# mitenjain/nanopore

Hardware: AMD Instinct MI355X
Metric: DP cells/sec (banded pair-HMM realign: forward + backward + posterior per cell) (higher is better)
Workload: dtype f32

## Files before the change

### nanopore_amd/csrc/npr_api.cpp

```cpp
#include "npr_api_internal.h"

namespace npr_impl {
DeviceArena g_arena[kMaxDevices];
}

extern "C" {

int32_t npr_abi_version(void) { return NPR_ABI_VERSION; }

const char *npr_strerror(int32_t code) {
    switch (code) {
        case NPR_OK: return "ok";
        case NPR_ERR_INVALID: return "invalid argument or guide alignment not global";
        case NPR_ERR_ZERO_PROB: return "total probability is zero inside the band";
        case NPR_ERR_CAPACITY: return "output capacity exceeded";
        case NPR_ERR_MODEL: return "unsupported or malformed HMM";
        case NPR_ERR_NO_DEVICE: return "no usable gfx950 device (there is no CPU fallback)";
        case NPR_ERR_HIP: return "HIP runtime error";
        case NPR_ERR_BAND_TOO_WIDE: return "band wider than the kernels support";
        case NPR_ERR_NOMEM: return "out of memory";
        case NPR_ERR_STATE: return "call sequence violated";
        default: return "unknown error";
    }
}
// ... 34 lines not shown
    }
    npr_ctx *ctx = new (std::nothrow) npr_ctx;
    if (!ctx) return NPR_ERR_NOMEM;
    ctx->device = device_id;
    ctx->arena = &g_arena[device_id];
    {
        std::lock_guard<std::mutex> lock(ctx->arena->mu);
        ++ctx->arena->users;
    }
    ctx->cu_count = prop.multiProcessorCount;
    ctx->total_mem = prop.totalGlobalMem;
    ctx->host_threads = usable_cpus();
    int prio_lo = 0, prio_hi = 0;
    (void)hipDeviceGetStreamPriorityRange(&prio_lo, &prio_hi);
    for (int i = 0; i < npr_ctx::kSideStreams; ++i)
        if ((e = hipStreamCreateWithPriority(&ctx->side[i], hipStreamNonBlocking, prio_hi)) != hipSuccess ||
            (e = hipEventCreateWithFlags(&ctx->side_done[i], hipEventDisableTiming)) != hipSuccess) {
            say("npr_create: side stream allocation", e);
            npr_destroy(ctx);
            return NPR_ERR_HIP;
        }
    if ((e = hipStreamCreateWithFlags(&ctx->stream, hipStreamNonBlocking)) != hipSuccess ||
        (e = hipEventCreate(&ctx->ev0)) != hipSuccess || (e = hipEventCreate(&ctx->ev1)) != hipSuccess ||
        (e = hipMalloc(reinterpret_cast<void **>(&ctx->d_models), sizeof(DevModel) * NPR_MAX_MODELS)) != hipSuccess) {
        say("npr_create: stream/event/model allocation", e);
        npr_destroy(ctx);
        return NPR_ERR_HIP;
    }
    const int32_t rc = npr_set_hmm(ctx, 0, nullptr, nullptr);
    if (rc != NPR_OK) {
        if (err && errlen) std::snprintf(err, errlen, "npr_create: %s", ctx->last_error.c_str());
        npr_destroy(ctx);
        return rc;
    }
    *out = ctx;
    return NPR_OK;
}

void npr_destroy(npr_ctx *ctx) {
    if (!ctx) return;
    (void)hipSetDevice(ctx->device);
    ctx->cache_flush();
    if (ctx->d_models) (void)hipFree(ctx->d_models);
    if (ctx->arena) {
        std::lock_guard<std::mutex> lock(ctx->arena->mu);
        if (--ctx->arena->users == 0) {
            if (ctx->arena->F) (void)hipFree(ctx->arena->F - DeviceArena::kPad);
            ctx->arena->F = nullptr, ctx->arena->cells = 0, ++ctx->arena->epoch;
        }
    }
    if (ctx->arena_Fx) (void)hipFree(reinterpret_cast<char *>(ctx->arena_Fx) - npr_ctx::kArenaPad);
    if (ctx->pin_pairs) (void)hipHostFree(ctx->pin_pairs);
    if (ctx->pin_stage) (void)hipHostFree(ctx->pin_stage);
    delete ctx->mea;
    for (hipEvent_t ev : ctx->ops_events) (void)hipEventDestroy(ev);
    if (ctx->ev0) (void)hipEventDestroy(ctx->ev0);
    if (ctx->ev1) (void)hipEventDestroy(ctx->ev1);
    if (ctx->stream) (void)hipStreamDestroy(ctx->stream);
    for (int i = 0; i < npr_ctx::kSideStreams; ++i) {
        if (ctx->side[i]) (void)hipStreamDestroy(ctx->side[i]);
        if (ctx->side_done[i]) (void)hipEventDestroy(ctx->side_done[i]);
    }
    delete ctx;
}

const char *npr_last_error(npr_ctx *ctx) { return ctx ? ctx->last_error.c_str() : ""; }

}
namespace npr_impl {
int32_t release_scratch(npr_ctx *ctx, bool caches_only) {
    HIP_TRY(ctx, hipSetDevice(ctx->device));
    HIP_TRY(ctx, hipStreamSynchronize(ctx->stream));
    ctx->cache_flush();
    if (caches_only) return NPR_OK;
    if (ctx->arena) {
        std::lock_guard<std::mutex> lock(ctx->arena->mu);
        if (ctx->arena->F) (void)hipFree(ctx->arena->F - DeviceArena::kPad);
        ctx->arena->F = nullptr, ctx->arena->cells = 0, ++ctx->arena->epoch;
    }
    if (ctx->arena_Fx) (void)hipFree(reinterpret_cast<char *>(ctx->arena_Fx) - npr_ctx::kArenaPad);
    ctx->arena_Fx = nullptr, ctx->arena_fx_cells = 0;
    delete ctx->mea;
    ctx->mea = nullptr;
    ctx->packed_pool.clear();
    return NPR_OK;
}
}
extern "C" {

int32_t npr_ctx_option(npr_ctx *ctx, int32_t option, int64_t value) {
    if (!ctx) return NPR_ERR_INVALID;
    switch (option) {
        case NPR_OPT_OVERLAP: ctx->overlap = value == 2 ? 2 : (value != 0 ? 1 : 0); return NPR_OK;
        case NPR_OPT_RELEASE_SCRATCH: return release_scratch(ctx, value == 2);
        case 10: case 11: case 12: case 16: case 18: case 19: break;
        default:
            if (option > NPR_OPT_RELEASE_SCRATCH && option < NPR_OPT_COUNT) {
                ctx->opt[option] = value;
                return NPR_OK;
            }
    }
    return fail(ctx, NPR_ERR_INVALID, "npr_ctx_option: unknown option");
}

int32_t npr_set_hmm(npr_ctx *ctx, int32_t slot, const double *T25, const double *E80) {
    if (!ctx || slot < 0 || slot >= NPR_MAX_MODELS) return NPR_ERR_INVALID;
// ... 139 lines not shown
```

### nanopore_amd/csrc/npr_api_internal.h

```cpp
#pragma once
#include <hip/hip_runtime.h>

#include <algorithm>
#include <atomic>
#include <chrono>
#include <cmath>
#include <cstdio>
#include <cstdlib>
#include <cstring>
#include <exception>
#include <memory>
#include <mutex>
#include <new>
#include <numeric>
#include <string>
#include <thread>
#include <type_traits>
#include <vector>

#include "npr_device.h"
#include "npr_internal.h"
#include "npr_sched.h"
#include "npr_threads.h"

using namespace npr;

struct npr_plan {
    Plan plan;
};

namespace npr_impl {
struct MeaScratch;

struct DeviceArena {
    static constexpr size_t kPad = 1024;
    std::mutex mu;
    char *F = nullptr;
    std::atomic<size_t> cells{0};
    std::atomic<uint64_t> epoch{1};
    int users = 0;
};
constexpr int kMaxDevices = 64;
extern DeviceArena g_arena[kMaxDevices];
}
using namespace npr_impl;

struct npr_ctx {
    int device = -1;
    hipStream_t stream = nullptr;
    hipEvent_t ev0 = nullptr, ev1 = nullptr;
    static constexpr int kSideStreams = 6;
    hipStream_t side[kSideStreams] = {};
    hipEvent_t side_done[kSideStreams] = {};
    int cu_count = 0;
    size_t total_mem = 0;
    bool model_set[NPR_MAX_MODELS] = {};
    DevModel models[NPR_MAX_MODELS];
    DevModel *d_models = nullptr;
    std::string last_error;
    int host_threads = 1;
    DeviceArena *arena = nullptr;
    int overlap = 0;
    int64_t opt[NPR_OPT_COUNT] = {};
    static constexpr size_t kArenaPad = DeviceArena::kPad;
    float *arena_Fx = nullptr;
    size_t arena_fx_cells = 0;
    void *pin_pairs = nullptr;
    size_t pin_pairs_bytes = 0;
    std::vector<hipEvent_t> ops_events;
    struct HostWords {
        std::unique_ptr<uint32_t[]> p;
        int64_t cap = 0;
    };
    std::vector<HostWords> packed_pool;
    void *pin_stage = nullptr;
    size_t pin_stage_bytes = 0;
    MeaScratch *mea = nullptr;
    struct Cached {
        void *p;
        size_t bytes;
    };
    std::vector<Cached> cache;
    size_t cache_bytes = 0;
    void cache_flush() {
        for (const Cached &c : cache) (void)hipFree(c.p);
        cache.clear();
        cache_bytes = 0;
    }
};

namespace npr_impl {

inline int poison_byte() {
    const char *e = std::getenv("NPR_POISON");
    return e && e[0] ? static_cast<int>(std::strtol(e, nullptr, 0)) & 0xff : -1;
}
inline void poison(void *p, size_t bytes) {
    if (poison_byte() >= 0 && p && bytes) {
        (void)hipMemset(p, poison_byte(), bytes);
        (void)hipDeviceSynchronize();
    }
}

template <typename T>
struct DevBuf {
    T *p = nullptr;
    size_t count = 0, cap = 0;
    hipError_t alloc(size_t n) {
        release();
        count = n;
        if (n == 0) return hipSuccess;
        const hipError_t e = hipMalloc(reinterpret_cast<void **>(&p), n * sizeof(T));
        if (e == hipSuccess) poison(p, n * sizeof(T));
        return e;
    }
    void release() {
        if (p && !borrowed) {
            if (owner && owner->cache.size() < 160) {
                owner->cache.push_back(npr_ctx::Cached{p, held});
                owner->cache_bytes += held;
            } else {
                (void)hipFree(p);
            }
        }
        p = nullptr;
        count = 0, cap = 0, borrowed = false, owner = nullptr, held = 0;
    }
    bool borrowed = false;
    void borrow(T *ptr, size_t n) {
        release();
        p = ptr, count = n, borrowed = true;
    }
    size_t bytes() const { return count * sizeof(T); }
    npr_ctx *owner = nullptr;
    size_t held = 0;
    hipError_t alloc_from(npr_ctx *ctx, size_t n) {
        release();
        count = n;
        if (n == 0) return hipSuccess;
        const size_t need = n * sizeof(T);
        constexpr size_t kSmall = size_t(1) << 20, kPiece = size_t(256) << 10;
        int best = -1;
        for (size_t i = 0; i < ctx->cache.size(); ++i)
            if (ctx->cache[i].bytes >= need && (ctx->cache[i].bytes <= 2 * need || ctx->cache[i].bytes <= kSmall) &&
                (best < 0 || ctx->cache[i].bytes < ctx->cache[best].bytes))
                best = static_cast<int>(i);
        if (best >= 0) {
            p = static_cast<T *>(ctx->cache[best].p), held = ctx->cache[best].bytes, owner = ctx;
            ctx->cache_bytes -= held;
            ctx->cache.erase(ctx->cache.begin() + best);
            poison(p, held);
            return hipSuccess;
        }
        const size_t take = need < kSmall ? (need + kPiece - 1) / kPiece * kPiece : need + need / 8;
        hipError_t e = hipMalloc(reinterpret_cast<void **>(&p), take);
        if (e != hipSuccess && !ctx->cache.empty()) {
            (void)hipGetLastError();
            ctx->cache_flush();
            e = hipMalloc(reinterpret_cast<void **>(&p), take);
        }
        if (e == hipSuccess) held = take, owner = ctx, poison(p, take);
        return e;
    }
    hipError_t reserve(size_t n) {
        if (n <= cap && p) {
            count = n;
            return hipSuccess;
        }
        const hipError_t e = alloc(n + n / 4 + 1);
        cap = e == hipSuccess ? count : 0;
        count = e == hipSuccess ? n : 0;
        return e;
    }
    ~DevBuf() { release(); }
};

struct MeaScratch {
    DevBuf<int64_t> off, mass, od;
    DevBuf<int32_t> cnt, start, col, sorted, small, tmp, map, pieces;
    DevBuf<uint32_t> dense;
};

inline int32_t fail(npr_ctx *ctx, int32_t code, const char *what, hipError_t e = hipSuccess) {
    if (code == NPR_ERR_HIP && e == hipErrorOutOfMemory) code = NPR_ERR_NOMEM, (void)hipGetLastError();
    if (ctx) {
        ctx->last_error = what;
        if (e != hipSuccess) {
            ctx->last_error += ": ";
            ctx->last_error += hipGetErrorString(e);
        }
    }
    return code;
}

#define HIP_TRY(ctx, expr)                                                  \
    do {                                                                    \
        hipError_t _e = (expr);                                             \
        if (_e != hipSuccess) return fail((ctx), NPR_ERR_HIP, #expr, _e);   \
    } while (0)

struct StageTimer {
    bool on;
    std::chrono::steady_clock::time_point t0;
    const char *what;
    explicit StageTimer(const char *w) : on(std::getenv("NPR_TIMING") != nullptr), t0(std::chrono::steady_clock::now()), what(w) {}
    void lap(const char *label) {
        if (!on) return;
        const auto t1 = std::chrono::steady_clock::now();
        std::fprintf(stderr, "[npr timing] %s / %s: %.1f ms\n", what, label, std::chrono::duration<double, std::milli>(t1 - t0).count());
        t0 = t1;
    }
};

}
using namespace npr_impl;

struct npr_batch {
    npr_ctx *ctx = nullptr;
    npr_params params{};
    int64_t n_reads = 0;
    std::vector<int64_t> ref_len, read_len;
    std::vector<int64_t> gstart;
    std::vector<int32_t> ref_id;
    std::vector<int32_t> guide_ops;
    std::vector<int64_t> guide_off;
    std::vector<int32_t> read_status;
    std::vector<int32_t> read_first_task, read_ntasks;
    std::vector<Task> tasks;
    std::vector<int32_t> task_of;
    std::vector<int64_t> task_cells;
    std::vector<TaskOut> outs;
    std::vector<uint8_t> task_rerun;
// ... 167 lines not shown
```

### nanopore_amd/csrc/npr_device.h

```cpp
#pragma once
#include <cstdint>

#include "npr_internal.h"
#include "npr_band.h"

namespace npr {

struct Task {
    int64_t x_off;
    int64_t y_off;
    int64_t band_off;
    int64_t pair_off;
    int32_t lX, lY;
    int32_t D;
    int32_t pair_cap;
    int32_t flags;
    int32_t model;
    int32_t xs, ys;
    int32_t read;
    int32_t cells_pad;
    int64_t ctl_off;
    int64_t tile_off;
    int64_t rowmask_off;
};
// ... 56 lines not shown
    const int32_t *px;
    const int32_t *py;
    const float *pp;
    int32_t *cx;
    int32_t *cy;
    float *cp;
};

int launch_generic(const KernelArgs &a, int grid, int threads, size_t lds_bytes, bool dense, bool global_ring, void *stream);
int launch_em(const KernelArgs &a, int grid, size_t lds_bytes, bool global_ring, void *stream);
size_t em_extra_lds_bytes();
int launch_compact(const CompactArgs &a, void *stream);
int launch_stair(const KernelArgs &a, int R, int grid, void *stream);
int launch_wide(const KernelArgs &a, int R, int NW, int grid, void *stream);
int launch_em_stair(const KernelArgs &a, int R, int grid, void *stream);
size_t em_stair_lds_bytes();
struct MeaArgs {
    const Task *tasks;
    const TaskOut *outs;
    int32_t ntasks, n_reads;
    const int32_t *px, *py;
    const float *pp;
    const int64_t *rx_off;
    const int64_t *ry_off;
    const int64_t *rp_off;
    int32_t *cnt, *start, *colsum;
    int32_t *sx, *sy, *sq, *back;
    int32_t *kx, *ky, *kq, *kback;
    int4 *vrec;
    int32_t *kept;
    const int32_t *np, *poff, *pboff, *lane_read, *lane_piece;
    int32_t *pb, *pbest;
    int32_t n_pieces;
    int32_t *best_who;
    int32_t *read_flag;
    double gap_gamma, match_gamma;
    int32_t ring;
    const int32_t *order;
    const int32_t *read_first, *read_ntasks, *task_of;
    int32_t sort_lds_bytes;
    int32_t sort_threads;
    int32_t any_global_sort;
    const int64_t *cnt_off;
    int32_t ring_only;
    int32_t *ops_tmp;
    const int64_t *ot_off;
    int32_t *n_ops, *chain_len;
    int64_t *chain_mass;
    uint32_t *ops_dense;
    const int64_t *od_off;
    int32_t *max_run;
    uint16_t *ops_dense16;
};
int launch_tile(const KernelArgs &a, int R, int NW, int grid, void *stream, bool flat = false);
size_t tile_lds_bytes(int nw);
int64_t tile_scratch_cells(int64_t rows, int R);
struct PlanSeg {
    int64_t point_first;
    int64_t band_off;
    int32_t pieces, lX, lY, pad;
};
struct SegSummary {
    int64_t cells;
    int64_t generic_cells;
    int32_t max_width;
    int32_t bad;
    int32_t rough;
    int32_t pad;
};
constexpr int kSchedClasses = 7;
constexpr int kSchedR[kSchedClasses] = {1, 2, 4, 2, 2, 4, 4};
constexpr int kSchedNW[kSchedClasses] = {1, 1, 1, 4, 8, 8, 12};
struct PlanArgs {
    int32_t n_segs, fixed_mode, width;
    const PlanPoint *points;
    const PlanSeg *segs;
    int32_t *lo, *n;
    SegSummary *summary;
};
struct SchedArgs {
    int32_t n_segs;
    const PlanSeg *segs;
    const SegSummary *summary;
    const int32_t *lo, *n;
    const int64_t *ctl_off;
    const uint32_t *cand;
    uint32_t *ctl;
    int32_t *cls;
    int64_t *cells;
};
struct StripeArgs {
    int32_t count, R;
    const int32_t *seg_index;
    const PlanSeg *segs;
    const SegSummary *summary;
    const int32_t *lo, *n;
    const int64_t *tile_off;
    Stripe *stripes;
    int64_t *rows;
};
struct CoffArgs {
    int32_t n_segs;
    const PlanSeg *segs;
    const int32_t *n;
    uint32_t *coff;
};
// ... 171 lines not shown
```

### nanopore_amd/csrc/npr_finish.cpp

```cpp
#include "npr_api_internal.h"

extern "C" {

}
namespace npr_impl {

int32_t fetch_pairs(npr_batch *b) {
    npr_ctx *ctx = b->ctx;
    if (b->pairs_ready) return NPR_OK;
    StageTimer tm("fetch_pairs");
    const int64_t ntasks = static_cast<int64_t>(b->tasks.size());
    const std::vector<int64_t> &dst = b->task_dst;
    const int32_t *hx = nullptr, *hy = nullptr;
    const float *hp = nullptr;
    const int64_t total = ntasks ? dst[ntasks] : 0;
    if (total) {
        DevBuf<int64_t> d_dst;
        DevBuf<int32_t> d_cx, d_cy;
        DevBuf<float> d_cp;
        hipError_t e;
        if ((e = d_dst.alloc_from(ctx, ntasks + 1)) != hipSuccess || (e = d_cx.alloc_from(ctx, total)) != hipSuccess ||
            (e = d_cy.alloc_from(ctx, total)) != hipSuccess || (e = d_cp.alloc_from(ctx, total)) != hipSuccess)
            return fail(ctx, NPR_ERR_NOMEM, "npr_batch_finish: hipMalloc", e);
        HIP_TRY(ctx, hipMemcpyAsync(d_dst.p, dst.data(), d_dst.bytes(), hipMemcpyHostToDevice, ctx->stream));
// ... 139 lines not shown
    DevBuf<unsigned long long> d_sum;
    hipError_t e;
    if ((e = d_sum.alloc_from(ctx, n)) != hipSuccess) return fail(ctx, NPR_ERR_NOMEM, "npr_batch_finish: hipMalloc (rescore sums)", e);
    HIP_TRY(ctx, hipMemsetAsync(d_sum.p, 0, sizeof(unsigned long long) * n, ctx->stream));
    RescoreArgs ra{static_cast<int32_t>(n), static_cast<int32_t>(ntasks), nullptr, nullptr, b->d_rs_gx_off.p, b->d_rs_gy.p, b->d_tasks.p, b->d_outs.p,
                   b->d_px.p, b->d_py.p, b->d_pp.p, d_sum.p, b->rs_shift};
    const int rc = launch_rescore_sum(ra, ctx->stream);
    if (rc != 0) return fail(ctx, NPR_ERR_HIP, "k_rescore_sum launch", static_cast<hipError_t>(rc));
    std::vector<unsigned long long> sum(n);
    HIP_TRY(ctx, hipMemcpyAsync(sum.data(), d_sum.p, sizeof(unsigned long long) * n, hipMemcpyDeviceToHost, ctx->stream));
    HIP_TRY(ctx, hipStreamSynchronize(ctx->stream));
    score.assign(n, 0.0);
    for (int64_t i = 0; i < n; ++i)
        if (b->rs_columns[i] > 0) score[i] = std::ldexp(static_cast<double>(sum[i]), -b->rs_shift) / static_cast<double>(b->rs_columns[i]);
    return NPR_OK;
}

int32_t device_mea(npr_batch *b) {
    npr_ctx *ctx = b->ctx;
    std::unique_lock<std::mutex> arena_lock(ctx->arena->mu, std::defer_lock);
    if (!ctx->overlap) arena_lock.lock();
    ++ctx->arena->epoch;
    StageTimer tm("device_mea");
    const int64_t n = b->n_reads, ntasks = static_cast<int64_t>(b->tasks.size());
    std::vector<int64_t> rx(n + 1, 0), ry(n + 1, 0), rp(n + 1, 0), ot(n + 1, 0), od(n + 1, 0);
    for (int64_t i = 0; i < n; ++i) {
        const bool ok = b->results[i].status == NPR_OK;
        const int64_t lX = ok ? b->ref_len[i] : 0, lY = ok ? b->read_len[i] : 0, np = ok ? b->pair_off[i + 1] - b->pair_off[i] : 0;
        rx[i + 1] = rx[i] + lX + 1;
        ry[i + 1] = ry[i] + lY;
        rp[i + 1] = rp[i] + np;
        ot[i + 1] = ot[i] + 3 * std::min({np, lX, lY}) + 2;
    }
    const int ring = 8192;
    const int64_t total = rp[n];
    constexpr int64_t kMaxPieces = 64, kLanesWanted = 64 * 5 * 256;
    const int64_t kPiecePairs = std::min<int64_t>(2048, std::max<int64_t>(128, total / kLanesWanted));
    std::vector<int32_t> np(n);
    int64_t n_pieces = 0;
    for (int64_t i = 0; i < n; ++i) np[i] = static_cast<int32_t>(std::min(kMaxPieces, std::max<int64_t>(1, (rp[i + 1] - rp[i] + kPiecePairs - 1) / kPiecePairs))), n_pieces += np[i];
    if (!ctx->mea) ctx->mea = new MeaScratch;
    MeaScratch &m = *ctx->mea;
    hipError_t e;
    const int64_t lds_span = ctx->opt[NPR_OPT_MEA_GLOBAL_SORT] != 0 ? 0 : 16 * 1024;
    int64_t span = 0;
    std::vector<int64_t> cnt_off(n + 1, -1);
    int64_t cnt_total = 0;
    for (int64_t i = 0; i < n; ++i) {
        const int64_t sp = std::max(rx[i + 1] - rx[i], ry[i + 1] - ry[i]);
        if (sp <= lds_span) span = std::max(span, sp);
        else cnt_off[i] = cnt_total, cnt_total += rx[i + 1] - rx[i];
    }
    const bool sort_in_lds = cnt_total == 0;
    const size_t ntask_map = b->task_of.size();
    const size_t n_cnt = sort_in_lds ? 1 : static_cast<size_t>(cnt_total);
    {
        auto al = [](size_t bytes) { return (bytes + 255) & ~size_t(255); };
        const size_t need = al(8 * 5 * (n + 1)) + al(8 * n) + al(8 * (n + 1)) + 2 * al(4 * n_cnt) + al(4 * (ry[n] + 1)) + al(4 * (12 * total + 16)) +
                            al(4 * 6 * n) + al(4 * 2 * ot[n]) + al(4 * (3 * n + ntask_map)) + al(4 * ot[n]) + al(4 * (4 * n_pieces + 4 * n));
        const bool arena_fits = ctx->arena->F && need <= static_cast<size_t>(ctx->arena->cells.load()) * 8;
        bool in_arena = !ctx->overlap && arena_fits;
        for (;;) {
            char *cur = ctx->arena->F;
            if (in_arena && poison_byte() >= 0) {
                HIP_TRY(ctx, hipStreamSynchronize(ctx->stream));
                poison(ctx->arena->F, need);
            }
            auto take = [&](auto &buf, size_t count) -> hipError_t {
                using T = std::remove_pointer_t<decltype(buf.p)>;
                if (!in_arena) return buf.reserve(count);
                buf.borrow(reinterpret_cast<T *>(cur), count);
                cur += al(sizeof(T) * count);
                return hipSuccess;
            };
            if ((e = take(m.off, 5 * (n + 1))) == hipSuccess && (e = take(m.mass, n)) == hipSuccess && (e = take(m.od, n + 1)) == hipSuccess &&
                (e = take(m.cnt, n_cnt)) == hipSuccess && (e = take(m.start, n_cnt)) == hipSuccess && (e = take(m.col, ry[n] + 1)) == hipSuccess &&
                (e = take(m.sorted, 12 * total + 16)) == hipSuccess && (e = take(m.small, 6 * n)) == hipSuccess && (e = take(m.tmp, 2 * ot[n])) == hipSuccess &&
                (e = take(m.map, 3 * n + ntask_map)) == hipSuccess && (e = take(m.dense, ot[n])) == hipSuccess &&
                (e = take(m.pieces, 4 * n_pieces + 4 * n)) == hipSuccess)
                break;
            (void)hipGetLastError();
            if (!in_arena && ctx->overlap && arena_fits) {
                m.off.release(), m.mass.release(), m.od.release(), m.cnt.release(), m.start.release(), m.col.release(), m.sorted.release();
                m.small.release(), m.tmp.release(), m.map.release(), m.dense.release(), m.pieces.release();
                ctx->cache_flush();
                arena_lock.lock();
                if (!(ctx->arena->F && need <= static_cast<size_t>(ctx->arena->cells.load()) * 8)) return 1;
                ++ctx->arena->epoch;
                in_arena = true;
                continue;
            }
            return 1;
        }
    }
    HIP_TRY(ctx, hipMemcpyAsync(m.map.p, b->read_first_task.data(), sizeof(int32_t) * n, hipMemcpyHostToDevice, ctx->stream));
    HIP_TRY(ctx, hipMemcpyAsync(m.map.p + n, b->read_ntasks.data(), sizeof(int32_t) * n, hipMemcpyHostToDevice, ctx->stream));
    HIP_TRY(ctx, hipMemcpyAsync(m.map.p + 2 * n, b->task_of.data(), sizeof(int32_t) * ntask_map, hipMemcpyHostToDevice, ctx->stream));
    std::vector<int32_t> order(n);
    std::iota(order.begin(), order.end(), 0);
    std::stable_sort(order.begin(), order.end(), [&](int32_t x, int32_t y) { return rp[x + 1] - rp[x] > rp[y + 1] - rp[y]; });
    HIP_TRY(ctx, hipMemcpyAsync(m.map.p + 2 * n + ntask_map, order.data(), sizeof(int32_t) * n, hipMemcpyHostToDevice, ctx->stream));
    {
        std::vector<int32_t> tab(3 * n + 2 * n_pieces);
        int32_t *const t_np = tab.data(), *const t_poff = t_np + n, *const t_pboff = t_poff + n, *const t_lr = t_pboff + n, *const t_lp = t_lr + n_pieces;
        int64_t at = 0;
        for (int64_t k = 0; k < n; ++k) {
            const int32_t r = order[k];
            t_np[r] = np[r], t_poff[r] = static_cast<int32_t>(at), t_pboff[r] = static_cast<int32_t>(at + k);
            for (int32_t j = 0; j < np[r]; ++j) t_lr[at + j] = r, t_lp[at + j] = j;
            at += np[r];
        }
        HIP_TRY(ctx, hipMemcpyAsync(m.pieces.p, tab.data(), sizeof(int32_t) * tab.size(), hipMemcpyHostToDevice, ctx->stream));
    }
    std::vector<int64_t> offs(5 * (n + 1));
    std::copy(cnt_off.begin(), cnt_off.end(), offs.begin() + 4 * (n + 1));
    std::copy(rx.begin(), rx.end(), offs.begin());
    std::copy(ry.begin(), ry.end(), offs.begin() + (n + 1));
    std::copy(rp.begin(), rp.end(), offs.begin() + 2 * (n + 1));
    std::copy(ot.begin(), ot.end(), offs.begin() + 3 * (n + 1));
    HIP_TRY(ctx, hipMemcpyAsync(m.off.p, offs.data(), m.off.bytes(), hipMemcpyHostToDevice, ctx->stream));
    HIP_TRY(ctx, hipMemsetAsync(m.small.p, 0, m.small.bytes(), ctx->stream));
    MeaArgs a{};
    a.tasks = b->d_tasks.p, a.outs = b->d_outs.p, a.ntasks = static_cast<int32_t>(ntasks), a.n_reads = static_cast<int32_t>(n);
    a.px = b->d_px.p, a.py = b->d_py.p, a.pp = b->d_pp.p;
    a.rx_off = m.off.p, a.ry_off = m.off.p + (n + 1), a.rp_off = m.off.p + 2 * (n + 1), a.ot_off = m.off.p + 3 * (n + 1);
    a.cnt = m.cnt.p, a.start = m.start.p, a.colsum = m.col.p;
    a.sx = m.sorted.p, a.sy = m.sorted.p + total + 1, a.sq = m.sorted.p + 2 * (total + 1), a.back = m.sorted.p + 3 * (total + 1);
    a.kx = m.sorted.p + 4 * (total + 1), a.ky = m.sorted.p + 5 * (total + 1), a.kq = m.sorted.p + 6 * (total + 1), a.kback = m.sorted.p + 7 * (total + 1);
    a.vrec = reinterpret_cast<int4 *>(m.sorted.p + ((8 * (total + 1) + 3) & ~int64_t(3)));
    a.best_who = m.small.p, a.read_flag = m.small.p + n, a.n_ops = m.small.p + 2 * n, a.chain_len = m.small.p + 3 * n, a.kept = m.small.p + 4 * n, a.max_run = m.small.p + 5 * n;
    a.chain_mass = m.mass.p;
    a.np = m.pieces.p, a.poff = m.pieces.p + n, a.pboff = m.pieces.p + 2 * n, a.lane_read = m.pieces.p + 3 * n, a.lane_piece = m.pieces.p + 3 * n + n_pieces;
    a.pbest = m.pieces.p + 3 * n + 2 * n_pieces, a.pb = m.pieces.p + 3 * n + 3 * n_pieces, a.n_pieces = static_cast<int32_t>(n_pieces);
    a.gap_gamma = b->params.gap_gamma, a.match_gamma = b->params.match_gamma, a.ring = ring;
    a.ring_only = ctx->opt[NPR_OPT_MEA_RING_ONLY] != 0 ? 1 : 0;
    a.read_first = m.map.p, a.read_ntasks = m.map.p + n, a.task_of = m.map.p + 2 * n, a.order = m.map.p + 2 * n + ntask_map;
    a.sort_lds_bytes = static_cast<int32_t>(4 * span);
    a.sort_threads = ctx->overlap == 1 ? 512 : 0;
    a.any_global_sort = sort_in_lds ? 0 : 1;
    a.cnt_off = m.off.p + 4 * (n + 1);
    a.ops_tmp = m.tmp.p, a.od_off = m.od.p;
    int rc = launch_mea_sort(a, ctx->stream);
    if (rc == 0) rc = launch_mea_chain(a, ctx->stream);
    if (rc != 0) return fail(ctx, NPR_ERR_HIP, "MEA kernel launch", static_cast<hipError_t>(rc));
    std::vector<int32_t> small(6 * n);
    std::vector<int64_t> mass(n);
    HIP_TRY(ctx, hipMemcpyAsync(small.data(), m.small.p, m.small.bytes(), hipMemcpyDeviceToHost, ctx->stream));
    HIP_TRY(ctx, hipMemcpyAsync(mass.data(), m.mass.p, m.mass.bytes(), hipMemcpyDeviceToHost, ctx->stream));
    HIP_TRY(ctx, hipStreamSynchronize(ctx->stream));
    tm.lap("sort + chain + trace");
    const int32_t *flag = small.data() + n, *nops = small.data() + 2 * n, *clen = small.data() + 3 * n;
    int32_t longest = 0;
    for (int64_t i = 0; i < n; ++i)
        if (b->results[i].status == NPR_OK && flag[i] == NPR_ERR_CAPACITY) return 1;
    for (int64_t i = 0; i < n; ++i) {
        npr_read_result &r = b->results[i];
        if (r.status == NPR_OK && flag[i] != 0) r.status = flag[i];
        const int64_t k = r.status == NPR_OK ? nops[i] : 0;
        od[i + 1] = od[i] + k;
        if (k) longest = std::max(longest, small[5 * n + i]);
        r.n_ops = k;
        r.score = (r.status == NPR_OK && clen[i] > 0) ? static_cast<double>(mass[i]) / (static_cast<double>(clen[i]) * PROB_ONE) : 0.0;
    }
    b->ops_off = od;
    b->ops_words = 2 * od[n];
    if (ctx->opt[NPR_OPT_FINISH_TEXT] != 0) return device_mea_text(b, a, od, tm);
    b->have_pairs_form = false, b->have_packed_form = true;
    if (od[n] > b->packed_cap)
        for (size_t i = 0; i < ctx->packed_pool.size(); ++i)
            if (ctx->packed_pool[i].cap >= od[n]) {
                b->packed = std::move(ctx->packed_pool[i].p), b->packed_cap = ctx->packed_pool[i].cap;
                ctx->packed_pool.erase(ctx->packed_pool.begin() + static_cast<std::ptrdiff_t>(i));
                break;
            }
    if (od[n] > b->packed_cap) {
        b->packed.reset(new uint32_t[od[n] + od[n] / 8]);
        b->packed_cap = od[n] + od[n] / 8;
    }
    if (od[n]) {
        const bool narrow = longest < (1 << 14) && ctx->opt[NPR_OPT_MEA_WIDE_OPS] == 0 &&
                            sizeof(uint16_t) * static_cast<size_t>(od[n]) <= m.sorted.bytes();
        a.ops_dense = m.dense.p;
        a.ops_dense16 = narrow ? reinterpret_cast<uint16_t *>(m.sorted.p) : nullptr;
        HIP_TRY(ctx, hipMemcpyAsync(m.od.p, od.data(), m.od.bytes(), hipMemcpyHostToDevice, ctx->stream));
        if ((rc = launch_mea_gather(a, ctx->stream)) != 0) return fail(ctx, NPR_ERR_HIP, "k_mea_gather launch", static_cast<hipError_t>(rc));
        const size_t word = narrow ? sizeof(uint16_t) : sizeof(uint32_t), need = word * static_cast<size_t>(od[n]);
        if (need > ctx->pin_pairs_bytes) {
            if (ctx->pin_pairs) (void)hipHostFree(ctx->pin_pairs);
            ctx->pin_pairs = nullptr, ctx->pin_pairs_bytes = 0;
            if ((e = hipHostMalloc(&ctx->pin_pairs, need + need / 4, hipHostMallocDefault)) != hipSuccess)
                return fail(ctx, NPR_ERR_NOMEM, "npr_batch_finish: hipHostMalloc", e);
// ... 318 lines not shown
```

### nanopore_amd/csrc/npr_mea.hip

```cpp
#include <hip/hip_runtime.h>

#include "npr_device.h"

namespace npr {
namespace {

constexpr int64_t P1 = PROB_ONE;
constexpr int WAVE = 64;
constexpr int SORT_THREADS = 1024;

__device__ __forceinline__ int rdlane(int v, int j) { return __builtin_amdgcn_readlane(v, j); }
__device__ __forceinline__ int64_t rdlane64(int64_t v, int j) {
    const int lo = __builtin_amdgcn_readlane(static_cast<int>(v), j);
    const int hi = __builtin_amdgcn_readlane(static_cast<int>(v >> 32), j);
    return (static_cast<int64_t>(hi) << 32) | static_cast<uint32_t>(lo);
}
__device__ __forceinline__ void wave_sync() {
    __builtin_amdgcn_fence(__ATOMIC_RELEASE, "wavefront");
    __builtin_amdgcn_wave_barrier();
    __builtin_amdgcn_fence(__ATOMIC_ACQUIRE, "wavefront");
}
__device__ __forceinline__ bool beats(int64_t s, int w, int64_t os, int ow) { return s > os || (s == os && w > ow); }

__device__ __forceinline__ int mea_task_pairs(const TaskOut &o, const Task &tk) { return o.status == NPR_OK ? min(max(o.npairs, 0), tk.pair_cap) : 0; }
// ... 22 lines not shown
                a.read_flag[r] = NPR_ERR_INVALID;
                continue;
            }
            const int q = static_cast<int>(floor(static_cast<double>(a.pp[tk.pair_off + i]) * static_cast<double>(P1)));
            atomicAdd(a.cnt + rx + x, 1);
            atomicAdd(a.colsum + ry + y, q);
        }
    }
}

__global__ void __launch_bounds__(256) k_mea_scan(MeaArgs a) {
    __shared__ int wsum[4];
    const int r = blockIdx.x, tid = threadIdx.x, lane = tid & 63, wv = tid >> 6;
    const int64_t rx = a.cnt_off[r];
    if (rx < 0) return;
    const int n = static_cast<int>(a.rx_off[r + 1] - a.rx_off[r]);
    int carry = 0;
    for (int base = 0; base < n; base += 256) {
        const int i = base + tid;
        const int v = i < n ? a.cnt[rx + i] : 0;
        int s = v;
        for (int o = 1; o < WAVE; o <<= 1) {
            const int t = __shfl_up(s, o);
            if (lane >= o) s += t;
        }
        if (lane == WAVE - 1) wsum[wv] = s;
        __syncthreads();
        int before = 0, total = 0;
        for (int k = 0; k < 4; ++k) before += k < wv ? wsum[k] : 0, total += wsum[k];
        if (i < n) a.start[rx + i] = carry + before + s - v;
        carry += total;
        __syncthreads();
    }
}

__global__ void __launch_bounds__(256) k_mea_scatter(MeaArgs a) {
    for (int t = blockIdx.x; t < a.ntasks; t += gridDim.x) {
        const Task &tk = a.tasks[t];
        const int n = mea_task_pairs(a.outs[t], tk);
        const int r = tk.read;
        const int64_t rx = a.cnt_off[r], rp = a.rp_off[r];
        if (rx < 0) continue;
        const int lX = static_cast<int>(a.rx_off[r + 1] - a.rx_off[r]) - 1, lY = static_cast<int>(a.ry_off[r + 1] - a.ry_off[r]);
        for (int i = threadIdx.x; i < n; i += blockDim.x) {
            const int x = a.px[tk.pair_off + i], y = a.py[tk.pair_off + i];
            if (x < 0 || x >= lX || y < 0 || y >= lY || !mea_is_posterior(a.pp[tk.pair_off + i])) continue;
            const int q = static_cast<int>(floor(static_cast<double>(a.pp[tk.pair_off + i]) * static_cast<double>(P1)));
            const int64_t pos = rp + a.start[rx + x] + (atomicSub(a.cnt + rx + x, 1) - 1);
            a.sx[pos] = x, a.sy[pos] = y, a.sq[pos] = q;
        }
    }
}

__global__ void __launch_bounds__(SORT_THREADS) k_mea_sort_lds(MeaArgs a) {
    extern __shared__ int h[];
    __shared__ int wsum[SORT_THREADS / WAVE];
    const int r = a.order[blockIdx.x], tid = threadIdx.x, lane = tid & 63, wv = tid >> 6;
    const int nthreads = static_cast<int>(blockDim.x);
    const int64_t rx = a.rx_off[r], ry = a.ry_off[r], rp = a.rp_off[r];
    const int lX = static_cast<int>(a.rx_off[r + 1] - rx) - 1, lY = static_cast<int>(a.ry_off[r + 1] - ry);
    if (a.rp_off[r + 1] == rp || a.cnt_off[r] >= 0) return;
    const int ft = a.read_first[r], nt = a.read_ntasks[r];
    int bad = 0;
    auto for_pairs = [&](auto f) {
        for (int s = 0; s < nt; ++s) {
            const int t = a.task_of[ft + s];
            const Task &tk = a.tasks[t];
            const int n = mea_task_pairs(a.outs[t], tk);
            for (int i = tid; i < n; i += nthreads) {
                const int x = a.px[tk.pair_off + i], y = a.py[tk.pair_off + i];
                if (x < 0 || x >= lX || y < 0 || y >= lY || !mea_is_posterior(a.pp[tk.pair_off + i])) {
                    bad = 1;
                    continue;
                }
                f(x, y, static_cast<int>(floor(static_cast<double>(a.pp[tk.pair_off + i]) * static_cast<double>(P1))));
            }
        }
    };
    for (int i = tid; i < lY; i += nthreads) h[i] = 0;
    __syncthreads();
    for_pairs([&](int, int y, int q) { atomicAdd(&h[y], q); });
    __syncthreads();
    for (int i = tid; i < lY; i += nthreads) a.colsum[ry + i] = h[i];
    __syncthreads();
    for (int i = tid; i <= lX; i += nthreads) h[i] = 0;
    __syncthreads();
    for_pairs([&](int x, int, int) { atomicAdd(&h[x], 1); });
    __syncthreads();
    int carry = 0;
    for (int base = 0; base <= lX; base += nthreads) {
        const int i = base + tid;
        const int v = i <= lX ? h[i] : 0;
        int sc = v;
        for (int o = 1; o < WAVE; o <<= 1) {
            const int t = __shfl_up(sc, o);
            if (lane >= o) sc += t;
        }
        if (lane == WAVE - 1) wsum[wv] = sc;
        __syncthreads();
        int before = 0, total = 0;
        for (int k = 0; k < nthreads / WAVE; ++k) before += k < wv ? wsum[k] : 0, total += wsum[k];
        if (i <= lX) h[i] = carry + before + sc - v;
        carry += total;
        __syncthreads();
    }
    for_pairs([&](int x, int y, int q) {
        const int64_t pos = rp + atomicAdd(&h[x], 1);
        a.sx[pos] = x, a.sy[pos] = y, a.sq[pos] = q;
    });
    if (bad) a.read_flag[r] = NPR_ERR_INVALID;
}

constexpr int MEA_RETRY = 1;

struct Chunk {
    int valid;
    uint64_t ends;
    uint64_t keep;
    int y, q;
    int64_t w;
    int who;
};
__device__ __forceinline__ Chunk prep_chunk(const MeaArgs &a, int *sx, int *sy, int *sq, int64_t ry, int base, int n, int lane,
                                            int64_t floor_w, int64_t *tw, int *ty, int *tq) {
    Chunk c;
    const int pos = base + lane;
    const bool in = pos < n;
    const int x = in ? sx[pos] : -1, xn = pos + 1 < n ? sx[pos + 1] : -2;
    int y = in ? sy[pos] : 0, q = in ? sq[pos] : 0;
    const uint64_t ends = __ballot(in && x != xn);
    c.valid = ends ? 64 - __builtin_clzll(ends) : 0;
    c.ends = ends, c.keep = 0, c.y = 0, c.q = 0, c.w = 0;
    if (!ends) return c;
    const bool act = lane < c.valid;
    const uint64_t starts = (ends << 1) | 1ull;
    const int gfirst = 63 - __builtin_clzll(starts & (lane == 63 ? ~0ull : ((2ull << lane) - 1)));
    const int gend = act ? lane + __builtin_ctzll(ends >> lane) : lane;
    const int gsize = gend - gfirst + 1;
    int rank = 0, rowsum = q;
    for (int o = 1; __any(act && o < gsize); ++o) {
        const int lo = lane - o, hi = lane + o;
        const int yl = __shfl(y, lo & 63), ql = __shfl(q, lo & 63), yh = __shfl(y, hi & 63), qh = __shfl(q, hi & 63);
        if (lo >= gfirst) rank += yl < y ? 1 : 0, rowsum += ql;
        if (hi <= gend) rank += yh < y ? 1 : 0, rowsum += qh;
    }
// ... 484 lines not shown
```

Measured before the change: 371.2 billion.

## Fuse MEA sort histogram passes and batch host uploads through pinned buffer

Adds a two-table mode to the LDS sort kernel. When both tables fit the per-workgroup LDS budget and the read has fewer than 65536 pairs, the column-sum and packed 16-bit row-count histograms are built in a single pass over the pairs. The separate second counting pass and its zeroing are skipped. The several small host-to-device copies of offsets, maps, order and piece tables are merged into one pinned staging buffer sent with a single memcpy, which drops the separate map buffer. The sort kernel's thread count is now set explicitly and its LDS size is computed per read, at the cost of a more complex LDS budgeting heuristic and 16-bit counters that limit per-read pair counts.

```diff
diff --git a/nanopore_amd/csrc/npr_api.cpp b/nanopore_amd/csrc/npr_api.cpp
--- a/nanopore_amd/csrc/npr_api.cpp
+++ b/nanopore_amd/csrc/npr_api.cpp
@@ -110,6 +110,7 @@
     if (ctx->arena_Fx) (void)hipFree(reinterpret_cast<char *>(ctx->arena_Fx) - npr_ctx::kArenaPad);
     if (ctx->pin_pairs) (void)hipHostFree(ctx->pin_pairs);
     if (ctx->pin_stage) (void)hipHostFree(ctx->pin_stage);
+    if (ctx->pin_mea) (void)hipHostFree(ctx->pin_mea);
     delete ctx->mea;
     for (hipEvent_t ev : ctx->ops_events) (void)hipEventDestroy(ev);
     if (ctx->ev0) (void)hipEventDestroy(ctx->ev0);
diff --git a/nanopore_amd/csrc/npr_api_internal.h b/nanopore_amd/csrc/npr_api_internal.h
--- a/nanopore_amd/csrc/npr_api_internal.h
+++ b/nanopore_amd/csrc/npr_api_internal.h
@@ -76,6 +76,8 @@
     void *pin_stage = nullptr;
     size_t pin_stage_bytes = 0;
     MeaScratch *mea = nullptr;
+    void *pin_mea = nullptr;
+    size_t pin_mea_bytes = 0;
     struct Cached {
         void *p;
         size_t bytes;
@@ -177,7 +179,7 @@
 
 struct MeaScratch {
     DevBuf<int64_t> off, mass, od;
-    DevBuf<int32_t> cnt, start, col, sorted, small, tmp, map, pieces;
+    DevBuf<int32_t> cnt, start, col, sorted, small, tmp, pieces;
     DevBuf<uint32_t> dense;
 };
 
diff --git a/nanopore_amd/csrc/npr_device.h b/nanopore_amd/csrc/npr_device.h
--- a/nanopore_amd/csrc/npr_device.h
+++ b/nanopore_amd/csrc/npr_device.h
@@ -132,6 +132,13 @@
     int32_t *max_run;
     uint16_t *ops_dense16;
 };
+constexpr int64_t kMeaSortTwoTable = -2;
+constexpr int64_t kMeaPackedPairs = 65536;
+constexpr int kMeaSortThreads = 1024;
+constexpr int kMeaSortStaticLds = 64;
+constexpr int kLdsBytesPerCu = 160 * 1024, kLdsGranule = 1280;
+NPR_HD constexpr int64_t mea_sort2_counts_at(int64_t lX, int64_t lY) { return lY > (lX + 2) / 2 ? lY : (lX + 2) / 2; }
+NPR_HD constexpr int64_t mea_sort2_words(int64_t lX, int64_t lY) { return mea_sort2_counts_at(lX, lY) + (lX + 2) / 2; }
 int launch_tile(const KernelArgs &a, int R, int NW, int grid, void *stream, bool flat = false);
 size_t tile_lds_bytes(int nw);
 int64_t tile_scratch_cells(int64_t rows, int R);
diff --git a/nanopore_amd/csrc/npr_finish.cpp b/nanopore_amd/csrc/npr_finish.cpp
--- a/nanopore_amd/csrc/npr_finish.cpp
+++ b/nanopore_amd/csrc/npr_finish.cpp
@@ -215,12 +215,30 @@
         else cnt_off[i] = cnt_total, cnt_total += rx[i + 1] - rx[i];
     }
     const bool sort_in_lds = cnt_total == 0;
+    const int sort_threads = ctx->overlap == 1 ? 512 : npr::kMeaSortThreads;
+    int64_t sort_lds_bytes = 0;
+    {
+        const int64_t granules_per_cu = npr::kLdsBytesPerCu / npr::kLdsGranule;
+        const int64_t granules_now = (4 * span + npr::kMeaSortStaticLds + npr::kLdsGranule - 1) / npr::kLdsGranule;
+        const int64_t wgs = std::max<int64_t>(1, std::min<int64_t>(2 * npr::kMeaSortThreads / sort_threads, granules_per_cu / granules_now));
+        const int64_t budget = granules_per_cu / wgs * npr::kLdsGranule - npr::kMeaSortStaticLds;
+        for (int64_t i = 0; i < n; ++i) {
+            if (cnt_off[i] >= 0) continue;
+            const int64_t lX = rx[i + 1] - rx[i] - 1, lY = ry[i + 1] - ry[i];
+            const int64_t both = 4 * npr::mea_sort2_words(lX, lY);
+            const bool two = both <= budget && rp[i + 1] - rp[i] < npr::kMeaPackedPairs;
+            if (two) cnt_off[i] = npr::kMeaSortTwoTable;
+            sort_lds_bytes = std::max(sort_lds_bytes, two ? both : 4 * std::max(lX + 1, lY));
+        }
+    }
     const size_t ntask_map = b->task_of.size();
+    const size_t up_off = 5 * static_cast<size_t>(n + 1), up_map = (3 * static_cast<size_t>(n) + ntask_map + 1) / 2;
+    const size_t up_words = up_off + up_map + (3 * static_cast<size_t>(n) + 2 * static_cast<size_t>(n_pieces) + 1) / 2;
     const size_t n_cnt = sort_in_lds ? 1 : static_cast<size_t>(cnt_total);
     {
         auto al = [](size_t bytes) { return (bytes + 255) & ~size_t(255); };
-        const size_t need = al(8 * 5 * (n + 1)) + al(8 * n) + al(8 * (n + 1)) + 2 * al(4 * n_cnt) + al(4 * (ry[n] + 1)) + al(4 * (12 * total + 16)) +
-                            al(4 * 6 * n) + al(4 * 2 * ot[n]) + al(4 * (3 * n + ntask_map)) + al(4 * ot[n]) + al(4 * (4 * n_pieces + 4 * n));
+        const size_t need = al(8 * up_words) + al(8 * n) + al(8 * (n + 1)) + 2 * al(4 * n_cnt) + al(4 * (ry[n] + 1)) + al(4 * (12 * total + 16)) +
+                            al(4 * 6 * n) + al(4 * 2 * ot[n]) + al(4 * ot[n]) + al(4 * (2 * n_pieces + n));
         const bool arena_fits = ctx->arena->F && need <= static_cast<size_t>(ctx->arena->cells.load()) * 8;
         bool in_arena = !ctx->overlap && arena_fits;
         for (;;) {
@@ -236,16 +254,15 @@
                 cur += al(sizeof(T) * count);
                 return hipSuccess;
             };
-            if ((e = take(m.off, 5 * (n + 1))) == hipSuccess && (e = take(m.mass, n)) == hipSuccess && (e = take(m.od, n + 1)) == hipSuccess &&
+            if ((e = take(m.off, up_words)) == hipSuccess && (e = take(m.mass, n)) == hipSuccess && (e = take(m.od, n + 1)) == hipSuccess &&
                 (e = take(m.cnt, n_cnt)) == hipSuccess && (e = take(m.start, n_cnt)) == hipSuccess && (e = take(m.col, ry[n] + 1)) == hipSuccess &&
                 (e = take(m.sorted, 12 * total + 16)) == hipSuccess && (e = take(m.small, 6 * n)) == hipSuccess && (e = take(m.tmp, 2 * ot[n])) == hipSuccess &&
-                (e = take(m.map, 3 * n + ntask_map)) == hipSuccess && (e = take(m.dense, ot[n])) == hipSuccess &&
-                (e = take(m.pieces, 4 * n_pieces + 4 * n)) == hipSuccess)
+                (e = take(m.dense, ot[n])) == hipSuccess && (e = take(m.pieces, 2 * n_pieces + n)) == hipSuccess)
                 break;
             (void)hipGetLastError();
             if (!in_arena && ctx->overlap && arena_fits) {
                 m.off.release(), m.mass.release(), m.od.release(), m.cnt.release(), m.start.release(), m.col.release(), m.sorted.release();
-                m.small.release(), m.tmp.release(), m.map.release(), m.dense.release(), m.pieces.release();
+                m.small.release(), m.tmp.release(), m.dense.release(), m.pieces.release();
                 ctx->cache_flush();
                 arena_lock.lock();
                 if (!(ctx->arena->F && need <= static_cast<size_t>(ctx->arena->cells.load()) * 8)) return 1;
@@ -256,16 +273,28 @@
             return 1;
         }
     }
-    HIP_TRY(ctx, hipMemcpyAsync(m.map.p, b->read_first_task.data(), sizeof(int32_t) * n, hipMemcpyHostToDevice, ctx->stream));
-    HIP_TRY(ctx, hipMemcpyAsync(m.map.p + n, b->read_ntasks.data(), sizeof(int32_t) * n, hipMemcpyHostToDevice, ctx->stream));
-    HIP_TRY(ctx, hipMemcpyAsync(m.map.p + 2 * n, b->task_of.data(), sizeof(int32_t) * ntask_map, hipMemcpyHostToDevice, ctx->stream));
-    std::vector<int32_t> order(n);
-    std::iota(order.begin(), order.end(), 0);
-    std::stable_sort(order.begin(), order.end(), [&](int32_t x, int32_t y) { return rp[x + 1] - rp[x] > rp[y + 1] - rp[y]; });
-    HIP_TRY(ctx, hipMemcpyAsync(m.map.p + 2 * n + ntask_map, order.data(), sizeof(int32_t) * n, hipMemcpyHostToDevice, ctx->stream));
+    if (8 * up_words > ctx->pin_mea_bytes) {
+        if (ctx->pin_mea) (void)hipHostFree(ctx->pin_mea);
+        ctx->pin_mea = nullptr, ctx->pin_mea_bytes = 0;
+        const size_t take = 8 * (up_words + up_words / 4);
+        if ((e = hipHostMalloc(&ctx->pin_mea, take, hipHostMallocDefault)) != hipSuccess) return fail(ctx, NPR_ERR_NOMEM, "npr_batch_finish: hipHostMalloc", e);
+        ctx->pin_mea_bytes = take;
+    }
+    int64_t *const h_off = static_cast<int64_t *>(ctx->pin_mea);
+    int32_t *const h_map = reinterpret_cast<int32_t *>(h_off + up_off), *const h_tab = reinterpret_cast<int32_t *>(h_off + up_off + up_map);
+    std::copy(rx.begin(), rx.end(), h_off);
+    std::copy(ry.begin(), ry.end(), h_off + (n + 1));
+    std::copy(rp.begin(), rp.end(), h_off + 2 * (n + 1));
+    std::copy(ot.begin(), ot.end(), h_off + 3 * (n + 1));
+    std::copy(cnt_off.begin(), cnt_off.end(), h_off + 4 * (n + 1));
+    std::copy(b->read_first_task.begin(), b->read_first_task.begin() + n, h_map);
+    std::copy(b->read_ntasks.begin(), b->read_ntasks.begin() + n, h_map + n);
+    std::copy(b->task_of.begin(), b->task_of.end(), h_map + 2 * n);
+    int32_t *const order = h_map + 2 * n + ntask_map;
+    std::iota(order, order + n, 0);
+    std::stable_sort(order, order + n, [&](int32_t x, int32_t y) { return rp[x + 1] - rp[x] > rp[y + 1] - rp[y]; });
     {
-        std::vector<int32_t> tab(3 * n + 2 * n_pieces);
-        int32_t *const t_np = tab.data(), *const t_poff = t_np + n, *const t_pboff = t_poff + n, *const t_lr = t_pboff + n, *const t_lp = t_lr + n_pieces;
+        int32_t *const t_np = h_tab, *const t_poff = t_np + n, *const t_pboff = t_poff + n, *const t_lr = t_pboff + n, *const t_lp = t_lr + n_pieces;
         int64_t at = 0;
         for (int64_t k = 0; k < n; ++k) {
             const int32_t r = order[k];
@@ -273,15 +302,8 @@
             for (int32_t j = 0; j < np[r]; ++j) t_lr[at + j] = r, t_lp[at + j] = j;
             at += np[r];
         }
-        HIP_TRY(ctx, hipMemcpyAsync(m.pieces.p, tab.data(), sizeof(int32_t) * tab.size(), hipMemcpyHostToDevice, ctx->stream));
-    }
-    std::vector<int64_t> offs(5 * (n + 1));
-    std::copy(cnt_off.begin(), cnt_off.end(), offs.begin() + 4 * (n + 1));
-    std::copy(rx.begin(), rx.end(), offs.begin());
-    std::copy(ry.begin(), ry.end(), offs.begin() + (n + 1));
-    std::copy(rp.begin(), rp.end(), offs.begin() + 2 * (n + 1));
-    std::copy(ot.begin(), ot.end(), offs.begin() + 3 * (n + 1));
-    HIP_TRY(ctx, hipMemcpyAsync(m.off.p, offs.data(), m.off.bytes(), hipMemcpyHostToDevice, ctx->stream));
+    }
+    HIP_TRY(ctx, hipMemcpyAsync(m.off.p, h_off, 8 * up_words, hipMemcpyHostToDevice, ctx->stream));
     HIP_TRY(ctx, hipMemsetAsync(m.small.p, 0, m.small.bytes(), ctx->stream));
     MeaArgs a{};
     a.tasks = b->d_tasks.p, a.outs = b->d_outs.p, a.ntasks = static_cast<int32_t>(ntasks), a.n_reads = static_cast<int32_t>(n);
@@ -293,13 +315,14 @@
     a.vrec = reinterpret_cast<int4 *>(m.sorted.p + ((8 * (total + 1) + 3) & ~int64_t(3)));
     a.best_who = m.small.p, a.read_flag = m.small.p + n, a.n_ops = m.small.p + 2 * n, a.chain_len = m.small.p + 3 * n, a.kept = m.small.p + 4 * n, a.max_run = m.small.p + 5 * n;
     a.chain_mass = m.mass.p;
-    a.np = m.pieces.p, a.poff = m.pieces.p + n, a.pboff = m.pieces.p + 2 * n, a.lane_read = m.pieces.p + 3 * n, a.lane_piece = m.pieces.p + 3 * n + n_pieces;
-    a.pbest = m.pieces.p + 3 * n + 2 * n_pieces, a.pb = m.pieces.p + 3 * n + 3 * n_pieces, a.n_pieces = static_cast<int32_t>(n_pieces);
+    const int32_t *const d_map = reinterpret_cast<const int32_t *>(m.off.p + up_off), *const d_tab = reinterpret_cast<const int32_t *>(m.off.p + up_off + up_map);
+    a.np = d_tab, a.poff = d_tab + n, a.pboff = d_tab + 2 * n, a.lane_read = d_tab + 3 * n, a.lane_piece = d_tab + 3 * n + n_pieces;
+    a.pbest = m.pieces.p, a.pb = m.pieces.p + n_pieces, a.n_pieces = static_cast<int32_t>(n_pieces);
     a.gap_gamma = b->params.gap_gamma, a.match_gamma = b->params.match_gamma, a.ring = ring;
     a.ring_only = ctx->opt[NPR_OPT_MEA_RING_ONLY] != 0 ? 1 : 0;
-    a.read_first = m.map.p, a.read_ntasks = m.map.p + n, a.task_of = m.map.p + 2 * n, a.order = m.map.p + 2 * n + ntask_map;
-    a.sort_lds_bytes = static_cast<int32_t>(4 * span);
-    a.sort_threads = ctx->overlap == 1 ? 512 : 0;
+    a.read_first = d_map, a.read_ntasks = d_map + n, a.task_of = d_map + 2 * n, a.order = d_map + 2 * n + ntask_map;
+    a.sort_lds_bytes = static_cast<int32_t>(sort_lds_bytes);
+    a.sort_threads = sort_threads;
     a.any_global_sort = sort_in_lds ? 0 : 1;
     a.cnt_off = m.off.p + 4 * (n + 1);
     a.ops_tmp = m.tmp.p, a.od_off = m.od.p;
diff --git a/nanopore_amd/csrc/npr_mea.hip b/nanopore_amd/csrc/npr_mea.hip
--- a/nanopore_amd/csrc/npr_mea.hip
+++ b/nanopore_amd/csrc/npr_mea.hip
@@ -98,6 +98,7 @@
     }
 }
 
+static_assert(SORT_THREADS == kMeaSortThreads && SORT_THREADS / WAVE * sizeof(int) == kMeaSortStaticLds, "npr_device.h prices this kernel's LDS");
 __global__ void __launch_bounds__(SORT_THREADS) k_mea_sort_lds(MeaArgs a) {
     extern __shared__ int h[];
     __shared__ int wsum[SORT_THREADS / WAVE];
@@ -106,6 +107,8 @@
     const int64_t rx = a.rx_off[r], ry = a.ry_off[r], rp = a.rp_off[r];
     const int lX = static_cast<int>(a.rx_off[r + 1] - rx) - 1, lY = static_cast<int>(a.ry_off[r + 1] - ry);
     if (a.rp_off[r + 1] == rp || a.cnt_off[r] >= 0) return;
+    const bool two = a.cnt_off[r] == kMeaSortTwoTable;
+    int *const cw = h + mea_sort2_counts_at(lX, lY);
     const int ft = a.read_first[r], nt = a.read_ntasks[r];
     int bad = 0;
     auto for_pairs = [&](auto f) {
@@ -124,19 +127,26 @@
         }
     };
     for (int i = tid; i < lY; i += nthreads) h[i] = 0;
+    if (two)
+        for (int i = tid; i < (lX + 2) / 2; i += nthreads) cw[i] = 0;
     __syncthreads();
-    for_pairs([&](int, int y, int q) { atomicAdd(&h[y], q); });
+    if (two)
+        for_pairs([&](int x, int y, int q) { atomicAdd(&h[y], q), atomicAdd(&cw[x >> 1], 1 << ((x & 1) * 16)); });
+    else
+        for_pairs([&](int, int y, int q) { atomicAdd(&h[y], q); });
     __syncthreads();
     for (int i = tid; i < lY; i += nthreads) a.colsum[ry + i] = h[i];
     __syncthreads();
-    for (int i = tid; i <= lX; i += nthreads) h[i] = 0;
-    __syncthreads();
-    for_pairs([&](int x, int, int) { atomicAdd(&h[x], 1); });
-    __syncthreads();
+    if (!two) {
+        for (int i = tid; i <= lX; i += nthreads) h[i] = 0;
+        __syncthreads();
+        for_pairs([&](int x, int, int) { atomicAdd(&h[x], 1); });
+        __syncthreads();
+    }
     int carry = 0;
     for (int base = 0; base <= lX; base += nthreads) {
         const int i = base + tid;
-        const int v = i <= lX ? h[i] : 0;
+        const int v = i > lX ? 0 : two ? (cw[i >> 1] >> ((i & 1) * 16)) & 0xffff : h[i];
         int sc = v;
         for (int o = 1; o < WAVE; o <<= 1) {
             const int t = __shfl_up(sc, o);
```

Result: no change. 374.0 billion, median of 6 (+0.7%).
